# scalar-labs/jepsen

Measured on AMD Instinct MI355X. Metric: history ops verified/sec (node), independent cas-register 10k keys, 1/2/4/8 GPU, higher is better.
Workload: dtype int64

## Files before the change

include/jh.h:

```cpp
#ifndef JH_H
#define JH_H

#include <stddef.h>
#include <stdint.h>

#ifdef __cplusplus
extern "C" {
#endif

#define JH_ABI_VERSION 8

#define JH_OK            0
#define JH_EINVAL        1
#define JH_EUNSUPPORTED  2
#define JH_EDEVICE       3
#define JH_ENOMEM        4

#define JH_TYPE_INVOKE 0
#define JH_TYPE_OK     1
#define JH_TYPE_FAIL   2
#define JH_TYPE_INFO   3

#define JH_F_READ  0
#define JH_F_WRITE 1
// ... 48 lines not shown
#define JH_LIN_INTERN_PER_KEY  4
#define JH_LIN_NO_HELPERS      8
#define JH_LIN_HELPERS_NOW    16
#define JH_LIN_PHASE1_ONLY    32
#define JH_LIN_SKIP_PHASE1    64
#define JH_LIN_NO_HANDOVER   128
#define JH_LIN_STREAM        256
#define JH_LIN_NO_RESUME     512
#define JH_LIN_EXACT_COUNT  1024
#define JH_EXPLORED_UNCOUNTED (-3)
#define JH_LIN_NO_SPEC      2048
#define JH_LIN_SPEC_FIRST   4096
#define JH_LIN_HELP_STALL   8192
#define JH_LIN_NO_TAKEOVER  16384
#define JH_LIN_TAKEOVER     32768

typedef struct jh_lin_opts {
    int64_t init_value;
    int64_t budget;
    int64_t stream;
    int32_t algorithm;
    int32_t flags;
    int64_t quick_budget;
    int64_t phase2_budget;
    int32_t helpers;
    int32_t helper_late_us;
    int32_t xw_waves;
    int32_t p2_waves_per_cu;
    int32_t lean_waves;
    int32_t wide_waves;
// ... 328 lines not shown
```

jepsen_amd/_abi.py:

```python
import ctypes as C

JH_ABI_VERSION = 8

JH_OK, JH_EINVAL, JH_EUNSUPPORTED, JH_EDEVICE, JH_ENOMEM = 0, 1, 2, 3, 4
TYPE_INVOKE, TYPE_OK, TYPE_FAIL, TYPE_INFO = 0, 1, 2, 3
F_READ, F_WRITE, F_CAS, F_ADD = 0, 1, 2, 3
F_ENQUEUE, F_DEQUEUE, F_DRAIN = 4, 5, 6
F_FIRST_INTERNED = 16
NIL = -(1 << 63)

VALID, UNKNOWN, INVALID = 0, 1, 2

CAUSES = {
    0: None,
    1: "budget",
    2: "window",
    3: "double-invoke",
    4: "orphan-completion",
    5: "unsupported-f",
    6: "nil-value",
    7: "overflow",
    8: "states",
    9: "deferred",
    10: "multiple-writes",
# ... 25 lines not shown

ALGO_COMPETITION, ALGO_WGL, ALGO_LINEAR = 0, 1, 2
ALGORITHMS = {"competition": ALGO_COMPETITION, "wgl": ALGO_WGL, "linear": ALGO_LINEAR}
LIN_BFS_ONLY, LIN_GEN_JUMP, LIN_INTERN_PER_KEY, LIN_NO_HELPERS, LIN_HELPERS_NOW = 1, 2, 4, 8, 16
LIN_PHASE1_ONLY, LIN_SKIP_PHASE1 = 32, 64
LIN_NO_HANDOVER = 128
LIN_STREAM = 256
LIN_NO_RESUME = 512
LIN_EXACT_COUNT = 1024
EXPLORED_UNCOUNTED = -3
LIN_NO_SPEC = 2048
LIN_SPEC_FIRST = 4096
LIN_HELP_STALL = 8192
LIN_NO_TAKEOVER = 16384
LIN_TAKEOVER = 32768
CAUSE_DEFERRED = 9


class JhLinOpts(C.Structure):
    _fields_ = [("init_value", C.c_int64), ("budget", C.c_int64), ("stream", C.c_int64),
                ("algorithm", C.c_int32), ("flags", C.c_int32),
                ("quick_budget", C.c_int64), ("phase2_budget", C.c_int64),
                ("helpers", C.c_int32), ("helper_late_us", C.c_int32),
                ("xw_waves", C.c_int32), ("p2_waves_per_cu", C.c_int32),
                ("lean_waves", C.c_int32), ("wide_waves", C.c_int32),
                ("handover_min", C.c_int32), ("p1_waves_per_cu", C.c_int32),
                ("bfs_wgs", C.c_int32), ("helper_stall_min", C.c_int32)]


VERDICT_FIELDS = ("valid", "cause", "fail_entry", "explored", "previous_ok", "last_op", "analyzer")
# ... 223 lines not shown
```

jepsen_amd/csrc/jh_lin.hip:

```cpp
#include "jh_internal.h"
#include <hipcub/hipcub.hpp>
#include <algorithm>
#include <type_traits>
#include "lin/lin_common.h"

namespace {

constexpr int F_READ = 0, F_WRITE = 1, F_CAS = 2, F_OTHER = 4;
constexpr int T_INVOKE = 0, T_OK = 1, T_FAIL = 2, T_INFO = 3;
constexpr uint64_t VIOL_NONE = ~0ULL;
#ifndef JH_LDS_TBL
#define JH_LDS_TBL 0
#endif
constexpr int LDS_TBL = JH_LDS_TBL;
#ifdef JH_STEP_PROF
#define PROF_MARK(v) const unsigned long long v = __builtin_amdgcn_s_memtime()
#define PROF_ADD(acc, a, b) acc += (b) - (a)
#else
#define PROF_MARK(v)
#define PROF_ADD(acc, a, b)
#endif
#ifdef JH_DFS_STATS
#define DFS_STAT(x) x
#else
// ... 59 lines not shown
struct RangeOut {
    long long vmin, vmax;
    long long pmax;
    int unkeyed_client;
    int bad_value;
    int smax;
    int pad;
};

__device__ __forceinline__ int f_code(int64_t f) {
    return f == JH_F_READ ? F_READ : f == JH_F_WRITE ? F_WRITE : f == JH_F_CAS ? F_CAS : F_OTHER;
}

__global__ void __launch_bounds__(256) k_range(const int64_t *__restrict__ proc, const int64_t *__restrict__ f,
                        const int64_t *__restrict__ key, const int64_t *__restrict__ v1,
                        const int64_t *__restrict__ v2, int64_t n, int keyed, RangeOut *out) {
    long long lo = LLONG_MAX, hi = LLONG_MIN, pm = -1;
    int unk = 0;
    for (int64_t r = blockIdx.x * (int64_t)blockDim.x + threadIdx.x; r < n;
         r += (int64_t)gridDim.x * blockDim.x) {
        int64_t p = proc[r];
        if (p < 0) continue;
        pm = max(pm, (long long)p);
        if (keyed && key && key[r] < 0) unk = 1;
        const int fc = f_code(f[r]);
        if (fc <= F_CAS) {
            int64_t a = v1[r];
            if (a != JH_NIL) { lo = min(lo, (long long)a); hi = max(hi, (long long)a); }
            if (fc == F_CAS) {
                int64_t b = v2[r];
                if (b != JH_NIL) { lo = min(lo, (long long)b); hi = max(hi, (long long)b); }
            }
        }
    }
    __shared__ long long sh[4];
    __shared__ int shi[4];
    lo = block_reduce256(lo, RedMin(), sh);
    hi = block_reduce256(hi, RedMax(), sh);
    pm = block_reduce256(pm, RedMax(), sh);
// ... 24 lines not shown
    while (a < b) {
        int64_t m = (a + b) >> 1;
        if (sk[m] < (uint32_t)k) a = m + 1; else b = m;
    }
    off[k] = (uint32_t)a;
    if (k < K) {
        int64_t a2 = a, b2 = n;
        while (a2 < b2) {
            int64_t m = (a2 + b2) >> 1;
            if (sk[m] <= (uint32_t)k) a2 = m + 1; else b2 = m;
        }
        atomicMax(&ro->smax, (int)(a2 - a));
    }
}

__global__ void k_gather(const int64_t *__restrict__ proc, const int64_t *__restrict__ type,
                         const int64_t *__restrict__ f, const int64_t *__restrict__ v1,
                         const int64_t *__restrict__ v2, const uint32_t *__restrict__ rows,
                         int64_t m, long long vmin, Rec *__restrict__ rec) {
    for (int64_t p = blockIdx.x * (int64_t)blockDim.x + threadIdx.x; p < m;
         p += (int64_t)gridDim.x * blockDim.x) {
        uint32_t r = rows[p];
        Rec x;
        int64_t pr = proc[r];
        x.proc = pr < 0 ? -1 : (int32_t)pr;
        x.type = (uint8_t)type[r];
        x.f = (uint8_t)f_code(f[r]);
        x.pad = 0;
        int64_t a = v1[r], b = v2[r];
        x.v1 = a == JH_NIL ? 0 : (int32_t)(a - vmin + 1);
        x.v2 = b == JH_NIL ? 0 : (int32_t)(b - vmin + 1);
        if (x.f > F_CAS) { x.v1 = 0; x.v2 = 0; }
        rec[p] = x;
    }
}

__global__ void __launch_bounds__(256) k_pair(const Rec *__restrict__ rec, const uint32_t *__restrict__ sk,
                                              const uint32_t *__restrict__ off, int64_t m,
                                              int32_t *__restrict__ pair,
                                              unsigned long long *__restrict__ viol) {
    const int lane = threadIdx.x & 63;
    const int64_t nw = (int64_t)gridDim.x * 4;
    for (int64_t wv = (int64_t)blockIdx.x * 4 + (threadIdx.x >> 6); wv * 64 < m; wv += nw) {
        const int64_t base = wv * 64, p = base + lane;
        int32_t xp = -1, xt = T_INFO;
        uint32_t k = 0;
        if (p < m) { const Rec x = rec[p]; xp = x.proc; xt = x.type; k = sk[p]; }
        const bool inv = p < m && xp >= 0 && xt == T_INVOKE;
        const int64_t end = inv ? (int64_t)off[k + 1] : 0;
        bool open = inv && end > p + 1;
        int64_t got = -1;
        int gtype = 0;
        for (int64_t wb = base; wb < m; wb += 64) {
            if (!__ballot(open)) break;
            const int64_t j = wb + lane;
            int32_t yp = -1, yt = T_INFO;
            uint32_t yk = 0xFFFFFFFFu;
            if (j < m) { const Rec y = rec[j]; yp = y.proc; yt = y.type; yk = sk[j]; }
            uint64_t todo = __ballot(open);
            while (todo) {
                const int l = __builtin_ctzll(todo);
                const int32_t pl = __builtin_amdgcn_readlane(xp, l);
                const uint32_t kl = (uint32_t)__builtin_amdgcn_readlane((int)k, l);
// ... 10 lines not shown
                        got = wb + b; gtype = (int)((cinv >> b) & 1); open = false;
                    }
                }
            }
            if (open && wb + 64 >= end) open = false;
        }
        if (got >= 0) {
            if (gtype) atomicMin(&viol[k], ((unsigned long long)got << 4) | JH_CAUSE_DOUBLE_INVOKE);
            else { pair[p] = (int32_t)got; pair[got] = (int32_t)p; }
        }
    }
}

__global__ void k_orphan(const Rec *__restrict__ rec, const uint32_t *__restrict__ sk,
                         int64_t m, const int32_t *__restrict__ pair,
                         unsigned long long *__restrict__ viol) {
    for (int64_t p = blockIdx.x * (int64_t)blockDim.x + threadIdx.x; p < m;
         p += (int64_t)gridDim.x * blockDim.x) {
        Rec x = rec[p];
        if (x.proc < 0 || (x.type != T_OK && x.type != T_FAIL)) continue;
        if (pair[p] < 0) atomicMin(&viol[sk[p]], ((unsigned long long)p << 4) | JH_CAUSE_ORPHAN);
    }
}

struct DfsArgs {
    const Rec *rec;
    const int32_t *pair;
    const uint32_t *off;
    const uint32_t *rows;
    const unsigned long long *viol;
    int32_t *rank;
    const int32_t *list;
    int32_t n_list;
    int32_t *queue;
    jh_key_verdict *out;
// ... 1757 lines not shown
struct TblArgs {
    KeySrc src;
    int64_t K;
    KeyMeta *meta;
    char *arena;
    unsigned long long *bump;
    jh_key_verdict *out;
    int32_t *list;
    int32_t *n_list;
    int32_t *list_w;
    int32_t *n_list_w;
    int32_t *list_x;
    int32_t *n_list_x;
    unsigned long long *xw_max;
    int32_t states8;
};

__global__ void __launch_bounds__(256) k_key_tables(TblArgs A) {
    const int lane = threadIdx.x & 63;
    const int64_t nw = (int64_t)gridDim.x * 4;
    for (int64_t key = (int64_t)blockIdx.x * 4 + (threadIdx.x >> 6); key < A.K; key += nw) {
        KeyInfo K;
        jh_key_verdict v;
        bool need = key_pass1(A.src, (int)key, lane, K, v);
        const bool long_key = K.n_ok >= COMPACT_MAX_OK || K.n_ops > 65535;
        if (need) {
            int maxw = 65;
            if (!long_key && K.sumW <= 64LL * K.n_ok) {
                unsigned long long off = 0;
                if (lane == 0) off = atomicAdd(A.bump, (unsigned long long)tblc_bytes(K));
                off = (unsigned long long)rfl64(__shfl(off, 0));
                maxw = key_fill_c<false>(A.src, K, lane, A.arena + off);
                if (maxw <= 64 && lane == 0) {
                    KeyMeta m;
                    m.off = off; m.n_ops = K.n_ops; m.n_ok = K.n_ok; m.maxw = maxw;
                    m.pad = (int32_t)min(K.sumW, (long long)0x7FFFFFFE);
                    A.meta[key] = m;
                    if (A.states8 && maxw <= 40) A.list[atomicAdd(A.n_list, 1)] = (int32_t)key;
                    else A.list_w[atomicAdd(A.n_list_w, 1)] = (int32_t)key;
                }
            }
            if (maxw > 64 && lane == 0) {
                KeyMeta m;
                m.off = 0; m.n_ops = K.n_ops; m.n_ok = K.n_ok; m.maxw = -1; m.pad = (int32_t)K.sumW;
                A.meta[key] = m;
                A.list_x[atomicAdd(A.n_list_x, 1)] = (int32_t)key;
                atomicMax(A.xw_max, (unsigned long long)xw_bytes(K.n_ops, K.n_ok, K.sumW));
            }
        }
        if (!need && lane == 0) A.out[key] = v;
    }
}

template <class M, bool LEAN, bool WL = false, bool STREAM = false, bool HO = false>
__device__ __forceinline__ void lin_dfs_waves(const DfsArgs &A) {
    const int lane = threadIdx.x;
    const size_t wv = (size_t)(blockIdx.x - A.wave_off);
    uint64_t *memo = A.memo + wv * A.memo_cap * 2;
    Frame *stack = A.stack + wv * A.stack_cap;
    uint64_t *stage = (uint64_t *)(A.scratch + wv * A.scratch_bytes);
    unsigned long long my_probes = 0;
    const int n_list = A.n_list_dev ? *A.n_list_dev : A.n_list;
    if (n_list < A.n_min || (A.n_max > 0 && n_list > A.n_max)) return;
    const unsigned long long t_begin = __builtin_amdgcn_s_memtime();
    bool spanned = false;
// ... 3605 lines not shown
    EV_EARLY_END = 11,
    EV_HELP_END = 12, EV_P3_START = 13,
};

struct KeyPartition {
    uint32_t *kA, *kB, *rA, *rB;
    uint32_t *off;
};
KeyPartition partition_buffers(jh_ctx *ctx, int64_t n) {
    KeyPartition p{};
    p.kA = ctx->ws<uint32_t>(WS_KEYS_A, n); p.kB = ctx->ws<uint32_t>(WS_KEYS_B, n);
    p.rA = ctx->ws<uint32_t>(WS_ROWS_A, n); p.rB = ctx->ws<uint32_t>(WS_ROWS_B, n);
    return p;
}
void partition_by_key(jh_ctx *ctx, KeyPartition &p, const int64_t *key, int64_t n, int64_t K, bool keyed,
                      RangeOut *ro, hipStream_t st) {
    if (n > 0)
        k_keys<<<grid_for(n, 256), 256, 0, st>>>(keyed ? key : nullptr, n, K, keyed ? 1 : 0, p.kA, p.rA);
    const int endbit = bits_for((uint64_t)K);
    size_t tb = 0;
    HIP_TRY(hipcub::DeviceRadixSort::SortPairs(nullptr, tb, p.kA, p.kB, p.rA, p.rB, (int)n, 0, endbit, st));
    void *tmp = ctx->ws<char>(WS_SORT_TMP, tb);
    HIP_TRY(hipcub::DeviceRadixSort::SortPairs(tmp, tb, p.kA, p.kB, p.rA, p.rB, (int)n, 0, endbit, st));
    if (!p.off) p.off = ctx->ws<uint32_t>(WS_SEG_OFF, K + 2);
    k_seg_off<<<grid_for(K + 1, 256), 256, 0, st>>>(p.kB, n, K, p.off, ro);
}

struct BfsSizes {
    uint32_t set_cap, q_cap;
};
BfsSizes bfs_table_sizes(int64_t reach_cap) {
    uint32_t set_cap = 1u << 12;
    while ((int64_t)set_cap < 2 * reach_cap && set_cap < (1u << 30)) set_cap <<= 1;
    const uint32_t q_cap = (uint32_t)std::min<int64_t>(reach_cap + 64, (int64_t)1 << 30);
    return BfsSizes{set_cap, q_cap};
}

struct LinRun {
    jh_ctx *ctx = nullptr;
    const jh_history *dh = nullptr;
// ... 2 lines not shown
    jh_key_verdict *out_dev = nullptr;
    jh_summary *sum = nullptr;
    hipStream_t st = nullptr;
    const LinCfgReq *cfgreq = nullptr;
    int64_t n = 0, K = 0, budget = 0, init = 0;
    int32_t lflags = 0;
    bool linear_mode = false;

    RangeOut *ro = nullptr;
    long long vmin = 0, vmax = 0, n_states = 0;
    bool per_key_values = false;
    int init_state = 0;
    uint32_t *kB = nullptr, *rB = nullptr, *off = nullptr;
    int64_t m = 0;
    int smax = 1;
    Rec *rec = nullptr;
    int32_t *pair = nullptr;
    unsigned long long *viol = nullptr;
    int32_t *rank = nullptr;

    uint32_t gen_span = 0;
    bool clear_memo = false;

    const uint32_t memo_cap1 = 1u << 16;
    int64_t quick = 0;
    int waves1 = 0;
    uint32_t stack_cap = 0;
    uint64_t scr_bytes = 0, scr_bytes_h = 0, scr_bytes_bfs = 0;
    uint64_t *memo = nullptr;
    Frame *stack = nullptr;
// ... 29 lines not shown
    int n_unres = 0;
    bool use_wg = false, wg_race = false, stream_p2 = false;
    int wg2 = 0, n_help = 0;
    BfsArgs c{};
    DfsArgs b{};
    WgArgs wr{}, wh{};
    unsigned long long *seq_start = nullptr;
    uint32_t *seq_stall = nullptr;
    int p2_per_cu = P2_LEAN_PER_CU;
    bool p2_m = true, bfs_only = false;

    KeySrc key_src() const { return KeySrc{rec, pair, off, rB, viol, rank, q + Q_FLAGS}; }

    void prepare();
    void prep_ranges();
    void prep_records();
    void intern_per_key();
    void memo_generation();
    void phase1_tables();
    void phase1_args();
    void phase1_resume();
    void phase2_budgets();
    void ensure_lds_attrs();
    void prep_xw(const int32_t *qw);
    void prep_wide();
    void launch_wide(hipStream_t sw, bool p2);
    WgArgs build_wg(int wg_cus, int32_t *wg_claim, int32_t *wg_queue, bool all_cus = false);
    void prep_race(int nd_all, int nd_l);
    void race_bfs(int nd_all);
    int race_helper_count(int nd_l);
    uint64_t *race_lean_sizing(int nd_l, int help_cus);
    void race_helpers(int nd_l);
    void race_lean_args(int nd_l, uint64_t *memo2);
    void timeline_tables(bool wide);
    DfsArgs phase1_wide_args() const;
    DfsArgs phase3_lean_args() const;
    DfsArgs phase3_wide_args() const;
    void launch_phase3_lean(int waves, hipStream_t s);
    void entry_lists(bool live);
    void record_no_heavy_keys();
    void run_streaming();
    void run_phase1();
    void sort_deferred();
// ... 11 lines not shown
    void diag_defer_timeline();
    void diag_acc_trace();
    void diag_ws_report();
    void diag_xw_prof();
    void diag_summary();
};

}

#include "lin/lin_diag.h"

namespace {

void LinRun::prep_ranges() {
    ro = ctx->ws<RangeOut>(WS_MISC, 1);
    RangeOut ro_init{LLONG_MAX, LLONG_MIN, -1, 0, 0, 0, 0};
    HIP_TRY(hipMemcpyAsync(ro, &ro_init, sizeof ro_init, hipMemcpyHostToDevice, st));
    if (n > 0)
        k_range<<<grid_for(n, 256, 4096), 256, 0, st>>>(dh->process, dh->f, keyed ? dh->key : nullptr,
                                                        dh->value, dh->value2, n, keyed ? 1 : 0, ro);
    RangeOut rh;
    HIP_TRY(hipMemcpyAsync(&rh, ro, sizeof rh, hipMemcpyDeviceToHost, st));
    HIP_TRY(hipStreamSynchronize(st));
    if (keyed && rh.unkeyed_client)
        throw_jh(JH_EUNSUPPORTED, "client ops whose :value is not an independent tuple");
    if (rh.pmax > INT32_MAX) throw_jh(JH_EUNSUPPORTED, "process ids beyond int32");
    vmin = rh.vmin; vmax = rh.vmax;
    if (init != JH_NIL) { vmin = std::min<long long>(vmin, init); vmax = std::max<long long>(vmax, init); }
    if (vmin > vmax) { vmin = 0; vmax = 0; }
    per_key_values = (unsigned long long)(vmax - vmin) >= (unsigned long long)(RQ_EMPTY - 3) ||
                     (lflags & JH_LIN_INTERN_PER_KEY) != 0;
    init_state = init == JH_NIL ? 0 : per_key_values ? 1 : (int)(init - vmin + 1);
    n_states = vmax - vmin + 2;
}

void LinRun::prep_records() {
    rec = ctx->ws<Rec>(WS_REC, m);
    pair = ctx->ws<int32_t>(WS_PAIR, m);
    viol = ctx->ws<unsigned long long>(WS_VIOL, K);
    rank = ctx->ws<int32_t>(WS_RANK, m);
    HIP_TRY(hipMemsetAsync(viol, 0xFF, sizeof(unsigned long long) * K, st));
    if (m > 0) {
        HIP_TRY(hipMemsetAsync(pair, 0xFF, sizeof(int32_t) * m, st));
        k_gather<<<grid_for(m, 256), 256, 0, st>>>(dh->process, dh->type, dh->f, dh->value, dh->value2,
                                                   rB, m, vmin, rec);
        k_pair<<<grid_for((m + 63) / 64, 4, 16384), 256, 0, st>>>(rec, kB, off, m, pair, viol);
        k_orphan<<<grid_for(m, 256), 256, 0, st>>>(rec, kB, m, pair, viol);
    }
}

void LinRun::intern_per_key() {
    const int64_t n2 = 2 * m;
    if (n2 >= (1LL << 32) - 1) throw_jh(JH_EUNSUPPORTED, "too many entries for per-key value interning");
    const int endbit = bits_for((uint64_t)K);
    uint64_t *iu = ctx->ws<uint64_t>(WS_IV_U, 2 * n2);
    uint32_t *ix = ctx->ws<uint32_t>(WS_IV_IDX, 3 * n2);
    uint32_t *ik = ctx->ws<uint32_t>(WS_IV_KEY, 2 * n2);
    uint32_t *rinit = ctx->ws<uint32_t>(WS_IV_RINIT, K + 1);
    unsigned int *maxid = (unsigned int *)ctx->ws<uint32_t>(WS_IV_MAX, 4);
    uint32_t *flag = ik + n2;
    k_ival<<<grid_for(n2, 256), 256, 0, st>>>(dh->value, dh->value2, dh->f, rB, m, iu, ix);
    size_t tb1 = 0, tb2 = 0, tb3 = 0;
// ... 10 lines not shown
    HIP_TRY(hipcub::DeviceScan::InclusiveSum(itmp, tb3, flag, flag, (int)n2, st));
    const uint64_t init_u = (uint64_t)init ^ (1ULL << 63);
    HIP_TRY(hipMemsetAsync(rinit, 0, sizeof(uint32_t) * (K + 1), st));
    HIP_TRY(hipMemsetAsync(maxid, 0, sizeof(unsigned int), st));
    if (init != JH_NIL) k_iinit<<<grid_for(n2, 256), 256, 0, st>>>(idx2, iu, kB, off, flag, n2, init_u, rinit);
    k_iassign<<<grid_for(n2, 256), 256, 0, st>>>(idx2, iu, kB, off, flag, n2, init != JH_NIL ? 1 : 0, init_u,
                                                 rinit, rec, viol, maxid);
    unsigned int mh = 0;
    HIP_TRY(hipMemcpyAsync(&mh, maxid, sizeof mh, hipMemcpyDeviceToHost, st));
    HIP_TRY(hipStreamSynchronize(st));
    n_states = (long long)std::max<unsigned int>(mh, init != JH_NIL ? 1u : 0u) + 1;
}

void LinRun::prepare() {
    prep_ranges();
    KeyPartition kp = partition_buffers(ctx, n);
    partition_by_key(ctx, kp, dh->key, n, K, keyed, ro, st);
    kB = kp.kB; rB = kp.rB; off = kp.off;
    uint32_t m_keyed = 0;
    RangeOut rh;
    HIP_TRY(hipMemcpyAsync(&m_keyed, off + K, sizeof m_keyed, hipMemcpyDeviceToHost, st));
    HIP_TRY(hipMemcpyAsync(&rh, ro, sizeof rh, hipMemcpyDeviceToHost, st));
    HIP_TRY(hipStreamSynchronize(st));
    m = m_keyed;
    smax = std::max(rh.smax, 1);
    prep_records();
    if (per_key_values && m > 0) intern_per_key();
}

void LinRun::memo_generation() {
    gen_span = (uint32_t)(3 * K + 3);
    clear_memo = false;
    if (lflags & JH_LIN_GEN_JUMP) ctx->gen_base = (1u << GEN_BITS) - 2;
    if ((uint64_t)ctx->gen_base + gen_span >= (1u << GEN_BITS) - 1) {
        ctx->gen_base = 0;
#ifndef JH_NO_WRAP_CLEAR
        clear_memo = true;
#endif
    }
}
// ... 6 lines not shown
    if (opts && opts->p1_waves_per_cu > 0) p1_per_cu = std::min(p1_per_cu, (int)opts->p1_waves_per_cu);
    waves1 = (int)std::min<int64_t>(K, (int64_t)ctx->n_cu * p1_per_cu);
    memo = ctx->ws<uint64_t>(WS_MEMO, (size_t)waves1 * memo_cap1 * 2, true);
    if (clear_memo) HIP_TRY(hipMemsetAsync(memo, 0, ctx->bufs[WS_MEMO].bytes, st));
    stack_cap = (uint32_t)smax + 2;
    stack = ctx->ws<Frame>(WS_STACK, (size_t)waves1 * stack_cap);
    scr_bytes = MemoQ::SLOTS * 8;
    scr_bytes_h = MemoH::SLOTS * 8;
    scr_bytes_bfs = (((uint64_t)smax * 84 + 4096) + 255) & ~255ULL;
    scr = ctx->ws<char>(WS_SCRATCH, (size_t)waves1 * scr_bytes);
    q = ctx->ws<int32_t>(WS_QUEUE, Q_WORDS);
    list = ctx->ws<int32_t>(WS_STATS, K);
    defer = ctx->ws<int32_t>(WS_DEFER, 3 * (size_t)(K + 1));
    defer_l = defer + (K + 1); defer_w = defer + 2 * (K + 1);
    d64 = ctx->ws<uint64_t>(WS_DEFER64, 3 * (size_t)(K + 1));
    HIP_TRY(hipMemsetAsync(q, 0, Q_WORDS * sizeof(int32_t), st));
    HIP_TRY(hipMemsetAsync(q + Q_T_WIDE, 0xFF, 2 * sizeof(int32_t), st));
    for (int w : {Q_T_BFS, Q_T_LEAN, Q_T_XW, Q_T_P1}) HIP_TRY(hipMemsetAsync(q + w, 0xFF, 2 * sizeof(int32_t), st));

    meta = ctx->ws<KeyMeta>(WS_META, K);
    arena = ctx->ws<char>(WS_ARENA, (size_t)m * 8 + (size_t)K * 32 + 256);
    TblArgs ta{};
    ta.src = key_src();
    ta.K = K; ta.meta = meta; ta.arena = arena; ta.bump = (unsigned long long *)(q + Q_BUMP);
    list_w = ctx->ws<int32_t>(WS_LIST_W, K);
    ta.out = out_dev; ta.list = list; ta.n_list = q + Q_N_LIST; ta.list_w = list_w; ta.n_list_w = q + Q_N_LIST_W;
    list_x = ctx->ws<int32_t>(WS_LIST_X, K);
    ta.list_x = list_x; ta.n_list_x = q + Q_N_LIST_X; ta.xw_max = (unsigned long long *)(q + Q_XW_MAX);
    ta.states8 = n_states <= 256 ? 1 : 0;
    k_key_tables<<<(unsigned)std::min<int64_t>((K + 3) / 4, 8192), 256, 0, st>>>(ta);

    list1 = list;
    if (!tune_env("JH_NO_LPT") && K > 1) {
        uint32_t *cost = ctx->ws<uint32_t>(WS_LCOST, 2 * K);
        int32_t *lv = ctx->ws<int32_t>(WS_LSORT, 2 * K);
        k_list_cost<<<grid_for(K, 256, 4096), 256, 0, st>>>(list, q + Q_N_LIST, meta, K, cost, lv);
        size_t tbl = 0;
        HIP_TRY(hipcub::DeviceRadixSort::SortPairsDescending(nullptr, tbl, cost, cost + K, lv, lv + K, (int)K, 0, 32, st));
        HIP_TRY(hipcub::DeviceRadixSort::SortPairsDescending(ctx->ws<char>(WS_LTMP, tbl), tbl, cost, cost + K, lv,
                                                             lv + K, (int)K, 0, 32, st));
        list1 = lv + K;
    }
}

void LinRun::phase1_args() {
// ... 222 lines not shown
    }
    wa.pend = ctx->ws<uint64_t>(WS_WG_PEND, (size_t)n_wg * 2 * work_cap);
    if (!ctx->lds_attr_wg) {
        HIP_TRY(hipFuncSetAttribute((const void *)k_lin_wg, hipFuncAttributeMaxDynamicSharedMemorySize, WG_LDS));
        ctx->lds_attr_wg = true;
    }
    return wa;
}

void LinRun::prep_race(int nd_all, int nd_l) {
    race_bfs(nd_all);
    const int help_cus = race_helper_count(nd_l);
    uint64_t *memo2 = race_lean_sizing(nd_l, help_cus);
    race_helpers(nd_l);
    race_lean_args(nd_l, memo2);
}

void LinRun::race_bfs(int nd_all) {
    claim = ctx->ws<int32_t>(WS_CLAIM, K);
    HIP_TRY(hipMemsetAsync(claim, 0, (size_t)K * sizeof(int32_t), st));
    HIP_TRY(hipMemsetAsync(q + Q_QUEUE, 0, sizeof(int32_t), st));
    HIP_TRY(hipMemsetAsync(q + Q_UNRES, 0, sizeof(int32_t), st));
    HIP_TRY(hipMemsetAsync(q + Q_P2_QUEUE, 0, sizeof(int32_t), st));

    uint32_t ncap = 1u << 22;
    if (const char *e = tune_env("JH_BFS_NODES")) ncap = (uint32_t)std::max(1 << 16, std::min(1 << 26, atoi(e)));
    const int64_t reach_cap = std::max<int64_t>(budget + 1, ncap);
    const BfsSizes sz = bfs_table_sizes(reach_cap);
    const uint32_t set_cap = sz.set_cap, q_cap = sz.q_cap;
    uint32_t hcap = 1u << 16;
    while (hcap < 2 * (uint64_t)ncap) hcap <<= 1;
    const uint32_t lcap = (uint32_t)smax + 2;
    const int bfs_cus = std::max(1, nd_all > 2000 && nd_all <= 4000 ? ctx->n_cu / 4
                                                                      : std::min(96, ctx->n_cu * 3 / 8));
    wg2 = std::min(nd_all, tune_env("JH_BFS_CUS") ? std::max(1, atoi(tune_env("JH_BFS_CUS"))) :
                           opts && opts->bfs_wgs > 0 ? std::min(opts->bfs_wgs, ctx->n_cu - 16) : bfs_cus);
    const uint64_t per_bfs = (uint64_t)set_cap * 8 + 4ULL * q_cap * 8 + scr_bytes_bfs + (uint64_t)ncap * 8 +
                             (uint64_t)lcap * 4 + (uint64_t)hcap * 16 + (uint64_t)ncap * 4 + ((uint64_t)ncap / 32 + 1) * 4 +
// ... 73 lines not shown
    }
    return memo2;
}

void LinRun::race_helpers(int nd_l) {
    wr = WgArgs{};
    if (wg_race && nd_l > 0) wr = build_wg(std::max(1, ctx->n_cu - wg2), claim, q + Q_P2_QUEUE);
    wh = WgArgs{};
    seq_start = nullptr;
    seq_stall = nullptr;
    if (n_help <= 0) return;
    const bool spec_on = !(lflags & JH_LIN_NO_SPEC) && !(tune_env("JH_SPEC") && !atoi(tune_env("JH_SPEC")));
    wh = build_wg(n_help, claim, nullptr, spec_on);
    seq_start = ctx->ws<unsigned long long>(WS_HELP_START, K);
    int32_t *taken = ctx->ws<int32_t>(WS_HELP_TAKEN, 2 * (size_t)K);
    HIP_TRY(hipMemsetAsync(seq_start, 0, (size_t)K * sizeof(unsigned long long), st));
    HIP_TRY(hipMemsetAsync(taken, 0, 2 * (size_t)K * sizeof(int32_t), st));
    seq_stall = (uint32_t *)(taken + K);
    wh.seq_start = seq_start; wh.seq_exit = q + Q_SEQ_EXIT; wh.seq_waves = waves2; wh.taken = taken;
    wh.mains_live = q + Q_MAINS;
    uint64_t late_us = HELPER_LATE_US;
    if (opts && opts->helper_late_us > 0) late_us = (uint64_t)opts->helper_late_us;
    if (lflags & JH_LIN_HELPERS_NOW) late_us = 0;
    wh.late_ticks = late_us * 100;
    const bool by_time = JH_HELP_BY_ORDER || (opts && opts->helper_late_us > 0) ||
                         (lflags & (JH_LIN_HELPERS_NOW | JH_LIN_HELP_STALL));
    wh.stall = by_time ? nullptr : seq_stall;
    wh.stall_min = opts && opts->helper_stall_min > 0 ? (uint32_t)opts->helper_stall_min : HELPER_STALL_MIN;
    if (spec_on) {
        wh.spec = ctx->ws<SpecSlot>(WS_SPEC, SPEC_SLOTS);
        HIP_TRY(hipMemsetAsync(wh.spec, 0, sizeof(SpecSlot) * SPEC_SLOTS, st));
        wh.spec_res_cap = SPEC_RES_CAP;
        wh.spec_res = ctx->ws<uint64_t>(WS_SPEC_RES, (size_t)n_wg * SPEC_RES_CAP);
        wh.spec_min = 512; wh.spec_mult = 32; wh.spec_dist = 128;
        wh.spec_q = q + Q_SPEC;
        wh.spec_first = (lflags & JH_LIN_SPEC_FIRST) ? 1 : 0;
        wh.n_mains = std::min(n_wg, HELPER_MAINS);
        if (const char *e = tune_env("JH_SPEC_SERVERS")) wh.n_mains = std::max(1, n_wg - std::max(0, atoi(e)));
        if (const char *e = tune_env("JH_SPEC_MIN")) wh.spec_min = (uint32_t)std::max(1, atoi(e));
        if (const char *e = tune_env("JH_SPEC_MULT")) wh.spec_mult = (uint32_t)std::max(1, atoi(e));
        if (const char *e = tune_env("JH_SPEC_DIST")) wh.spec_dist = (uint32_t)std::max(1, atoi(e));
    }
}

void LinRun::race_lean_args(int nd_l, uint64_t *memo2) {
    const int wmax = std::max(waves2, waves3);
// ... 7 lines not shown
    b.defer_list = defer3; b.defer_count = q + Q_DEFER3;
    b.defer64 = nullptr; b.defer_kind = nullptr; b.defer_kind_count = nullptr;
    b.memo = memo2; b.memo_cap = cap2l; b.stack = stack2; b.scratch = scr2; b.scratch_bytes = scr_bytes_h;
    b.budget = split3 ? p2 : budget;
    b.budget_full = split3 && cap2l == cap2 ? budget : 0;
    b.gen_base = ctx->gen_base + (uint32_t)K + 1;
    b.dbg = dbg ? dbg + 16 * 256 : nullptr; b.claim = claim;
    b.probes = (unsigned long long *)(q + Q_PROBES_SEQ);
    b.seq_start = seq_start; b.exit_count = seq_start ? q + Q_SEQ_EXIT : nullptr;
    b.stamp_progress = seq_start && (lflags & JH_LIN_HELP_STALL) ? 1 : 0;
    b.stall = seq_stall;
    b.defer_time = nullptr;
    b.handoff = nullptr;
    if (n_help > 0 && a.rs_off && waves2 > 0 && (lflags & JH_LIN_TAKEOVER) && !(lflags & JH_LIN_NO_TAKEOVER)) {
        int32_t *ho = ctx->ws<int32_t>(WS_HANDOFF, K);
        HIP_TRY(hipMemsetAsync(ho, 0, (size_t)K * sizeof(int32_t), st));
        b.handoff = ho;
        b.hlog_cap = 32768;
        b.hlog = ctx->ws<uint32_t>(WS_RS_LOG2, (size_t)wmax * b.hlog_cap);
        wh.d.handoff = ho;
    }
}

void LinRun::timeline_tables(bool wide) {
    if (!defer_times) return;
    unsigned long long *tl = ctx->ws<unsigned long long>(WS_TL, TL_W * (size_t)K);
    HIP_TRY(hipMemsetAsync(tl, 0, TL_W * sizeof(unsigned long long) * K, st));
    c.tl = tl; b.tl = tl;
    if (wide) bw.tl = tl;
    if (n_help > 0) wh.d.tl = tl;
}
// ... 552 lines not shown
```

Measured before the change: 261.3 million.

## Fuse per-key record gather, pairing and table build into one wave kernel

Adds k_key_build, a one-wave-per-key kernel that builds the records, pairs invocations with completions, checks violations and emits the key tables from LDS, for keys up to a segment cap. The separate gather/pair/orphan/tables kernels now run only on longer keys, or not at all. k_range also writes the key and row arrays for the partition step, and the many small hipMemsetAsync calls are batched into one fill kernel plus a queue-init kernel. The aim is to cut launch overhead and global-memory round trips during preparation, at the cost of a large and complex new code path that has to reproduce the old pairing semantics exactly.

Result: faster. 265.9 million (median of 6 runs) (+1.7%).

```diff
diff --git a/include/jh.h b/include/jh.h
--- a/include/jh.h
+++ b/include/jh.h
@@ -86,6 +86,8 @@
 #define JH_LIN_HELP_STALL   8192
 #define JH_LIN_NO_TAKEOVER  16384
 #define JH_LIN_TAKEOVER     32768
+#define JH_LIN_PREP_SPLIT   65536
+#define JH_LIN_PREP_CAP     1024
 
 typedef struct jh_lin_opts {
     int64_t init_value;
diff --git a/jepsen_amd/_abi.py b/jepsen_amd/_abi.py
--- a/jepsen_amd/_abi.py
+++ b/jepsen_amd/_abi.py
@@ -63,6 +63,8 @@
 LIN_HELP_STALL = 8192
 LIN_NO_TAKEOVER = 16384
 LIN_TAKEOVER = 32768
+LIN_PREP_SPLIT = 65536
+LIN_PREP_CAP = 1024
 CAUSE_DEFERRED = 9
 
 
diff --git a/jepsen_amd/csrc/jh_lin.hip b/jepsen_amd/csrc/jh_lin.hip
--- a/jepsen_amd/csrc/jh_lin.hip
+++ b/jepsen_amd/csrc/jh_lin.hip
@@ -97,15 +97,19 @@
 
 __global__ void __launch_bounds__(256) k_range(const int64_t *__restrict__ proc, const int64_t *__restrict__ f,
                         const int64_t *__restrict__ key, const int64_t *__restrict__ v1,
-                        const int64_t *__restrict__ v2, int64_t n, int keyed, RangeOut *out) {
+                        const int64_t *__restrict__ v2, int64_t n, int keyed, RangeOut *out,
+                        int64_t K, uint32_t *__restrict__ k32, uint32_t *__restrict__ r32) {
     long long lo = LLONG_MAX, hi = LLONG_MIN, pm = -1;
     int unk = 0;
     for (int64_t r = blockIdx.x * (int64_t)blockDim.x + threadIdx.x; r < n;
          r += (int64_t)gridDim.x * blockDim.x) {
         int64_t p = proc[r];
+        const int64_t kr = keyed ? (key ? key[r] : -1) : 0;
+        k32[r] = (kr >= 0 && kr < K) ? (uint32_t)kr : (uint32_t)K;
+        r32[r] = (uint32_t)r;
         if (p < 0) continue;
         pm = max(pm, (long long)p);
-        if (keyed && key && key[r] < 0) unk = 1;
+        if (keyed && key && kr < 0) unk = 1;
         const int fc = f_code(f[r]);
         if (fc <= F_CAS) {
             int64_t a = v1[r];
@@ -160,12 +164,18 @@
     }
 }
 
+__device__ __forceinline__ bool seg_longer(const uint32_t *off, uint32_t k, int64_t min_len) {
+    return (int64_t)(off[k + 1] - off[k]) > min_len;
+}
+
 __global__ void k_gather(const int64_t *__restrict__ proc, const int64_t *__restrict__ type,
                          const int64_t *__restrict__ f, const int64_t *__restrict__ v1,
                          const int64_t *__restrict__ v2, const uint32_t *__restrict__ rows,
-                         int64_t m, long long vmin, Rec *__restrict__ rec) {
+                         int64_t m, long long vmin, Rec *__restrict__ rec,
+                         const uint32_t *__restrict__ sk, const uint32_t *__restrict__ off, int64_t min_len) {
     for (int64_t p = blockIdx.x * (int64_t)blockDim.x + threadIdx.x; p < m;
          p += (int64_t)gridDim.x * blockDim.x) {
+        if (min_len >= 0 && !seg_longer(off, sk[p], min_len)) continue;
         uint32_t r = rows[p];
         Rec x;
         int64_t pr = proc[r];
@@ -184,7 +194,7 @@
 __global__ void __launch_bounds__(256) k_pair(const Rec *__restrict__ rec, const uint32_t *__restrict__ sk,
                                               const uint32_t *__restrict__ off, int64_t m,
                                               int32_t *__restrict__ pair,
-                                              unsigned long long *__restrict__ viol) {
+                                              unsigned long long *__restrict__ viol, int64_t min_len) {
     const int lane = threadIdx.x & 63;
     const int64_t nw = (int64_t)gridDim.x * 4;
     for (int64_t wv = (int64_t)blockIdx.x * 4 + (threadIdx.x >> 6); wv * 64 < m; wv += nw) {
@@ -192,7 +202,7 @@
         int32_t xp = -1, xt = T_INFO;
         uint32_t k = 0;
         if (p < m) { const Rec x = rec[p]; xp = x.proc; xt = x.type; k = sk[p]; }
-        const bool inv = p < m && xp >= 0 && xt == T_INVOKE;
+        const bool inv = p < m && xp >= 0 && xt == T_INVOKE && (min_len < 0 || seg_longer(off, k, min_len));
         const int64_t end = inv ? (int64_t)off[k + 1] : 0;
         bool open = inv && end > p + 1;
         int64_t got = -1;
@@ -233,11 +243,12 @@
 
 __global__ void k_orphan(const Rec *__restrict__ rec, const uint32_t *__restrict__ sk,
                          int64_t m, const int32_t *__restrict__ pair,
-                         unsigned long long *__restrict__ viol) {
+                         unsigned long long *__restrict__ viol, const uint32_t *__restrict__ off, int64_t min_len) {
     for (int64_t p = blockIdx.x * (int64_t)blockDim.x + threadIdx.x; p < m;
          p += (int64_t)gridDim.x * blockDim.x) {
         Rec x = rec[p];
         if (x.proc < 0 || (x.type != T_OK && x.type != T_FAIL)) continue;
+        if (min_len >= 0 && !seg_longer(off, sk[p], min_len)) continue;
         if (pair[p] < 0) atomicMin(&viol[sk[p]], ((unsigned long long)p << 4) | JH_CAUSE_ORPHAN);
     }
 }
@@ -2025,12 +2036,14 @@
     int32_t *n_list_x;
     unsigned long long *xw_max;
     int32_t states8;
+    int64_t min_len;
 };
 
 __global__ void __launch_bounds__(256) k_key_tables(TblArgs A) {
     const int lane = threadIdx.x & 63;
     const int64_t nw = (int64_t)gridDim.x * 4;
     for (int64_t key = (int64_t)blockIdx.x * 4 + (threadIdx.x >> 6); key < A.K; key += nw) {
+        if (A.min_len >= 0 && !seg_longer(A.src.off, (uint32_t)key, A.min_len)) continue;
         KeyInfo K;
         jh_key_verdict v;
         bool need = key_pass1(A.src, (int)key, lane, K, v);
@@ -2060,6 +2073,295 @@
             }
         }
         if (!need && lane == 0) A.out[key] = v;
+    }
+}
+
+constexpr int KB_CAP = JH_LIN_PREP_CAP;
+constexpr int KB_GATHER = 4;
+static_assert(KB_CAP < COMPACT_MAX_OK && KB_CAP < 32768 && KB_CAP < (int)T_MASK, "segment-local ranks and pairs");
+
+struct BuildArgs {
+    TblArgs t;
+    const int64_t *proc, *type, *f, *v1, *v2;
+    long long vmin;
+    Rec *rec;
+    int32_t *pair;
+    unsigned long long *viol;
+};
+
+struct KbLds {
+    int32_t pr[KB_CAP];
+    uint16_t v1[KB_CAP], v2[KB_CAP];
+    int16_t pw[KB_CAP];
+    int16_t ri[KB_CAP];
+    uint8_t tf[KB_CAP];
+};
+
+__device__ int kb_scan_back(const KbLds &sh, int pl, int base, int lane) {
+    for (int b = base - 64; b >= 0; b -= 64) {
+        const int ty = sh.tf[b + lane] & 31;
+        const uint64_t m = ballot(sh.pr[b + lane] == pl && ty != T_INFO);
+        if (m) {
+            const int h = 63 - __builtin_clzll(m);
+            return readlane(ty, h) == T_INVOKE ? b + h : -1;
+        }
+    }
+    return -1;
+}
+
+__device__ __forceinline__ void kb_settle(jh_key_verdict *out, int64_t key, int valid, int cause, long long explored) {
+    jh_key_verdict v{};
+    v.valid = valid; v.cause = cause; v.fail_entry = -1; v.explored = explored;
+    out[key] = v;
+}
+
+__device__ __forceinline__ uint32_t kb_rq(int f, int v1c, int v2c) {
+    return f == F_READ ? ((uint32_t)v1c | ((uint32_t)v1c << 16))
+         : f == F_WRITE ? (RQ_ANY | ((uint32_t)v1c << 16))
+         : ((uint32_t)v1c | ((uint32_t)v2c << 16));
+}
+
+__device__ __forceinline__ int wave_sum(int x) {
+    for (int o = 32; o > 0; o >>= 1) x += __shfl_xor(x, o);
+    return x;
+}
+
+__global__ void __launch_bounds__(64) k_key_build(BuildArgs B) {
+    __shared__ KbLds sh;
+    const int lane = threadIdx.x;
+    const uint64_t lt = (1ULL << lane) - 1;
+    const TblArgs &A = B.t;
+    const KeySrc &S = A.src;
+    const int64_t k8 = (A.K + 7) / 8;
+    for (int64_t b = blockIdx.x; b < 8 * k8; b += gridDim.x) {
+        const int64_t key = (b & 7) * k8 + (b >> 3);
+        if (key >= A.K) continue;
+        const uint32_t s0 = S.off[key], s1 = S.off[key + 1];
+        if (s1 - s0 > (uint32_t)KB_CAP) continue;
+        const int len = (int)(s1 - s0);
+        if (len == 0) {
+            if (lane == 0) { B.viol[key] = VIOL_NONE; kb_settle(A.out, key, JH_VALID, 0, -1); }
+            continue;
+        }
+        wave_sync();
+        for (int base = 0; base < len; base += 64 * KB_GATHER) {
+            uint32_t r[KB_GATHER];
+            int64_t cp[KB_GATHER], ct[KB_GATHER], cf[KB_GATHER], ca[KB_GATHER], cb[KB_GATHER];
+#pragma unroll
+            for (int g = 0; g < KB_GATHER; g++) r[g] = S.rows[s0 + min(base + g * 64 + lane, len - 1)];
+#pragma unroll
+            for (int g = 0; g < KB_GATHER; g++) {
+                cp[g] = B.proc[r[g]]; ct[g] = B.type[r[g]]; cf[g] = B.f[r[g]]; ca[g] = B.v1[r[g]]; cb[g] = B.v2[r[g]];
+            }
+#pragma unroll
+            for (int g = 0; g < KB_GATHER; g++) {
+                const int i = base + g * 64 + lane;
+                if (i >= len) continue;
+                Rec x;
+                x.proc = cp[g] < 0 ? -1 : (int32_t)cp[g];
+                x.type = (uint8_t)ct[g];
+                x.f = (uint8_t)f_code(cf[g]);
+                x.pad = 0;
+                x.v1 = ca[g] == JH_NIL ? 0 : (int32_t)(ca[g] - B.vmin + 1);
+                x.v2 = cb[g] == JH_NIL ? 0 : (int32_t)(cb[g] - B.vmin + 1);
+                if (x.f > F_CAS) { x.v1 = 0; x.v2 = 0; }
+                B.rec[s0 + i] = x;
+                sh.pr[i] = x.proc;
+                sh.v1[i] = (uint16_t)x.v1; sh.v2[i] = (uint16_t)x.v2;
+                sh.tf[i] = (uint8_t)((x.type > 31 ? 31 : x.type) | (x.f << 5));
+                sh.pw[i] = -1;
+            }
+        }
+        wave_sync();
+        unsigned long long vi = VIOL_NONE;
+        {
+            int tproc = 0, tpos = -1;
+            bool recycled = false;
+            int victim = 0;
+            for (int base = 0; base < len; base += 64) {
+                const int i = base + lane;
+                const bool valid = i < len;
+                const int xp = valid ? sh.pr[i] : -1;
+                const int xt = valid ? sh.tf[i] & 31 : T_INFO;
+                const bool cand = xp >= 0 && xt != T_INFO;
+                const uint64_t invm = ballot(cand && xt == T_INVOKE);
+                uint64_t mygrp = 0;
+                int mypred0 = -1;
+                uint64_t todo = ballot(cand);
+                while (todo) {
+                    const int pl = readlane(xp, __builtin_ctzll(todo));
+                    const bool mine = cand && xp == pl;
+                    const uint64_t grp = ballot(mine);
+                    todo &= ~grp;
+                    const uint64_t hit = ballot(tpos >= 0 && tproc == pl);
+                    int pred0 = -1;
+                    if (hit) {
+                        const int hl = __builtin_ctzll(hit);
+                        pred0 = readlane(tpos, hl);
+                        if (lane == hl) tpos = -1;
+                    } else if (recycled) {
+                        pred0 = kb_scan_back(sh, pl, base, lane);
+                    }
+                    if (mine) { mygrp = grp; mypred0 = pred0; }
+                    const int last = 63 - __builtin_clzll(grp);
+                    if ((invm >> last) & 1) {
+                        const uint64_t fr = ~ballot(tpos >= 0);
+                        int slot;
+                        if (fr) slot = __builtin_ctzll(fr);
+                        else { slot = victim; victim = (victim + 1) & 63; recycled = true; }
+                        if (lane == slot) { tproc = pl; tpos = base + last; }
+                    }
+                }
+                if (cand) {
+                    const uint64_t below = mygrp & lt;
+                    int pred = mypred0;
+                    bool pinv = mypred0 >= 0;
+                    if (below) {
+                        const int bl = 63 - __builtin_clzll(below);
+                        pred = base + bl; pinv = ((invm >> bl) & 1) != 0;
+                    }
+                    if (pinv && xt == T_INVOKE)
+                        vi = min(vi, ((unsigned long long)(s0 + i) << 4) | JH_CAUSE_DOUBLE_INVOKE);
+                    else if (pinv) { sh.pw[i] = (int16_t)pred; sh.pw[pred] = (int16_t)i; }
+                    else if (xt == T_OK || xt == T_FAIL)
+                        vi = min(vi, ((unsigned long long)(s0 + i) << 4) | JH_CAUSE_ORPHAN);
+                }
+            }
+            for (int o = 32; o > 0; o >>= 1) vi = min(vi, (unsigned long long)__shfl_xor((long long)vi, o));
+        }
+        wave_sync();
+        for (int base = 0; base < len; base += 64) {
+            const int i = base + lane;
+            if (i < len) {
+                const int q = sh.pw[i];
+                B.pair[s0 + i] = q < 0 ? -1 : (int32_t)(s0 + q);
+            }
+        }
+        if (lane == 0) B.viol[key] = vi;
+        if (vi != VIOL_NONE) {
+            if (lane == 0) kb_settle(A.out, key, JH_UNKNOWN, (int)(vi & 15), 0);
+            continue;
+        }
+        int n_ops = 0, n_ok = 0, n_crash = 0, badf = 0;
+        int acc_ok = 0, acc_crash = 0, acc_w = 0;
+        for (int base = 0; base < len; base += 64) {
+            const int i = base + lane;
+            const bool valid = i < len;
+            int xp = -1, xt = 0, xf = 0, xv1 = 0, xv2 = 0, q = -1;
+            if (valid) {
+                const int tf = sh.tf[i];
+                xp = sh.pr[i]; xt = tf & 31; xf = tf >> 5; xv1 = sh.v1[i]; xv2 = sh.v2[i]; q = sh.pw[i];
+            }
+            int yt = 0, yf = 0, yv1 = 0, yv2 = 0;
+            if (q >= 0) {
+                const int tf = sh.tf[q];
+                yt = tf & 31; yf = tf >> 5; yv1 = sh.v1[q]; yv2 = sh.v2[q];
+            }
+            const bool inv = xp >= 0 && xt == T_INVOKE;
+            const bool c_ok = inv && q >= 0 && yt == T_OK;
+            const bool c_fail = inv && q >= 0 && yt == T_FAIL;
+            int v1c = xv1;
+            if (c_ok && xv1 == 0 && (xf != F_CAS || xv2 == 0)) v1c = yv1;
+            const bool kept = inv && !c_fail && !(xf == F_READ && (!c_ok || v1c == 0));
+            bool ret = false;
+            if (xp >= 0 && xt == T_OK && q >= 0) {
+                int iv1 = yv1;
+                if (iv1 == 0 && (yf != F_CAS || yv2 == 0)) iv1 = xv1;
+                ret = !(yf == F_READ && iv1 == 0);
+            }
+            const uint64_t bi = ballot(kept), br = ballot(ret);
+            const int my_op = n_ops + mbcnt(bi);
+            const int a = n_ok + mbcnt(br);
+            const int rk = kept ? my_op : (ret ? -(a + 2) : -1);
+            if (valid) { S.rank[s0 + i] = rk; sh.pr[i] = rk; sh.ri[i] = (int16_t)(ret ? q : -1); }
+            badf |= (int)(ballot(kept && xf > F_CAS) != 0);
+            const bool crash = kept && !c_ok;
+            n_crash += __popcll(ballot(crash));
+            acc_ok += (kept && c_ok) ? a : 0;
+            acc_crash += crash ? a : 0;
+            if (ret) acc_w = max(acc_w, my_op - a);
+            n_ops += __popcll(bi);
+            n_ok += __popcll(br);
+        }
+        const int sum_a_ok = wave_sum(acc_ok), sum_a_crash = wave_sum(acc_crash);
+        int maxw = acc_w;
+        for (int o = 32; o > 0; o >>= 1) maxw = max(maxw, __shfl_xor(maxw, o));
+        KeyInfo K;
+        K.s0 = s0; K.s1 = s1; K.n_ops = n_ops; K.n_ok = n_ok;
+        K.sumW = (long long)n_ok * (n_ok + 1) / 2 - sum_a_ok + (long long)n_crash * n_ok - sum_a_crash;
+        const int cause = badf ? JH_CAUSE_BAD_F : n_ok == 0 ? 0 : K.sumW > (long long)JH_MAX_WINDOW * n_ok ? JH_CAUSE_WINDOW : -1;
+        if (cause >= 0) {
+            if (lane == 0) kb_settle(A.out, key, cause ? JH_UNKNOWN : JH_VALID, cause, 0);
+            continue;
+        }
+        if (maxw > 64) {
+            if (lane == 0) {
+                KeyMeta m;
+                m.off = 0; m.n_ops = n_ops; m.n_ok = n_ok; m.maxw = -1; m.pad = (int32_t)K.sumW;
+                A.meta[key] = m;
+                A.list_x[atomicAdd(A.n_list_x, 1)] = (int32_t)key;
+                atomicMax(A.xw_max, (unsigned long long)xw_bytes(n_ops, n_ok, K.sumW));
+            }
+            continue;
+        }
+        unsigned long long off = 0;
+        if (lane == 0) off = atomicAdd(A.bump, (unsigned long long)tblc_bytes(K));
+        off = (unsigned long long)rfl64(__shfl(off, 0));
+        OpC *ops = (OpC *)(A.arena + off);
+        Lay *lay = (Lay *)(A.arena + off + tblc_ops_bytes(K));
+        wave_sync();
+        int nok = 0, since = 0;
+        for (int base = 0; base < len; base += 64) {
+            const int i = base + lane;
+            const int rk = i < len ? sh.pr[i] : -1;
+            const bool kept = rk >= 0, ret = rk <= -2;
+            const uint64_t bi = ballot(kept), br = ballot(ret);
+            if (kept) {
+                const int xf = sh.tf[i] >> 5, q = sh.pw[i];
+                int rr = -1, v1c = sh.v1[i], v2c = sh.v2[i];
+                if (q >= 0 && (sh.tf[q] & 31) == T_OK) {
+                    rr = -(sh.pr[q] + 2);
+                    if (xf == F_CAS) { if (v1c == 0 && v2c == 0) { v1c = sh.v1[q]; v2c = sh.v2[q]; } }
+                    else if (v1c == 0) v1c = sh.v1[q];
+                }
+                const int a = nok + mbcnt(br);
+                OpC o;
+                o.rq = kb_rq(xf, v1c, v2c);
+                o.fa = (uint32_t)xf | ((uint32_t)a << 2) | ((uint32_t)(rr + 1) << 16);
+                ops[rk] = o;
+            }
+            if (ret) {
+                const int t = -(rk + 2), q = sh.pw[i];
+                const uint64_t rb = br & lt;
+                int c;
+                if (rb) c = __popcll(bi & lt & ~((2ULL << (63 - __builtin_clzll(rb))) - 1));
+                else c = since + __popcll(bi & lt);
+                int nested = 0;
+                for (int p2 = q + 1; p2 < i; p2 += 4) {
+                    const int r0 = sh.ri[p2], r1 = sh.ri[min(p2 + 1, i)], r2 = sh.ri[min(p2 + 2, i)], r3 = sh.ri[min(p2 + 3, i)];
+                    nested += (r0 > q) + (p2 + 1 < i && r1 > q) + (p2 + 2 < i && r2 > q) + (p2 + 3 < i && r3 > q);
+                }
+                const int r = sh.pr[q] - t + nested;
+                const int yf = sh.tf[q] >> 5;
+                int v1c = sh.v1[q], v2c = sh.v2[q];
+                if (yf == F_CAS) { if (v1c == 0 && v2c == 0) { v1c = sh.v1[i]; v2c = sh.v2[i]; } }
+                else if (v1c == 0) v1c = sh.v1[i];
+                Lay e;
+                e.rq = kb_rq(yf, v1c, v2c);
+                e.hi = (uint32_t)r | ((uint32_t)c << 6);
+                lay[t] = e;
+            }
+            since = br ? __popcll(bi & ~((2ULL << (63 - __builtin_clzll(br))) - 1)) : since + __popcll(bi);
+            nok += __popcll(br);
+        }
+        if (lane == 0) {
+            KeyMeta m;
+            m.off = off; m.n_ops = n_ops; m.n_ok = n_ok; m.maxw = maxw;
+            m.pad = (int32_t)min(K.sumW, (long long)0x7FFFFFFE);
+            A.meta[key] = m;
+            if (A.states8 && maxw <= 40) A.list[atomicAdd(A.n_list, 1)] = (int32_t)key;
+            else A.list_w[atomicAdd(A.n_list_w, 1)] = (int32_t)key;
+        }
     }
 }
 
@@ -5695,8 +5997,8 @@
     return p;
 }
 void partition_by_key(jh_ctx *ctx, KeyPartition &p, const int64_t *key, int64_t n, int64_t K, bool keyed,
-                      RangeOut *ro, hipStream_t st) {
-    if (n > 0)
+                      RangeOut *ro, hipStream_t st, bool have_pairs = false) {
+    if (n > 0 && !have_pairs)
         k_keys<<<grid_for(n, 256), 256, 0, st>>>(keyed ? key : nullptr, n, K, keyed ? 1 : 0, p.kA, p.rA);
     const int endbit = bits_for((uint64_t)K);
     size_t tb = 0;
@@ -5705,6 +6007,30 @@
     HIP_TRY(hipcub::DeviceRadixSort::SortPairs(tmp, tb, p.kA, p.kB, p.rA, p.rB, (int)n, 0, endbit, st));
     if (!p.off) p.off = ctx->ws<uint32_t>(WS_SEG_OFF, K + 2);
     k_seg_off<<<grid_for(K + 1, 256), 256, 0, st>>>(p.kB, n, K, p.off, ro);
+}
+
+__global__ void k_init_q(int32_t *q) {
+    const int w = threadIdx.x;
+    if (w >= Q_WORDS) return;
+    bool start = false;
+    for (int s : {Q_T_WIDE, Q_T_BFS, Q_T_LEAN, Q_T_XW, Q_T_P1}) start |= w == s || w == s + 1;
+    q[w] = start ? -1 : 0;
+}
+
+struct FillJob {
+    uint32_t *p;
+    uint64_t words;
+    uint32_t val;
+    uint32_t pad;
+};
+struct FillBatch {
+    FillJob j[8];
+    int n;
+};
+__global__ void __launch_bounds__(256) k_fill(FillBatch F) {
+    for (int i = 0; i < F.n; i++)
+        for (uint64_t w = blockIdx.x * 256ull + threadIdx.x; w < F.j[i].words; w += gridDim.x * 256ull)
+            F.j[i].p[w] = F.j[i].val;
 }
 
 struct BfsSizes {
@@ -5737,6 +6063,11 @@
     uint32_t *kB = nullptr, *rB = nullptr, *off = nullptr;
     int64_t m = 0;
     int smax = 1;
+    KeyPartition kp{};
+    FillBatch fills{};
+    const RangeOut ro_init{LLONG_MAX, LLONG_MIN, -1, 0, 0, 0, 0};
+    bool fused = false;
+    int64_t split_min = -1;
     Rec *rec = nullptr;
     int32_t *pair = nullptr;
     unsigned long long *viol = nullptr;
@@ -5796,6 +6127,7 @@
 
     void prepare();
     void prep_ranges();
+    void use_ranges(const RangeOut &rh);
     void prep_records();
     void intern_per_key();
     void memo_generation();
@@ -5809,6 +6141,8 @@
     void launch_wide(hipStream_t sw, bool p2);
     WgArgs build_wg(int wg_cus, int32_t *wg_claim, int32_t *wg_queue, bool all_cus = false);
     void prep_race(int nd_all, int nd_l);
+    void fill_later(void *p, size_t bytes, uint32_t val);
+    void flush_fills();
     void race_bfs(int nd_all);
     int race_helper_count(int nd_l);
     uint64_t *race_lean_sizing(int nd_l, int help_cus);
@@ -5850,14 +6184,14 @@
 
 void LinRun::prep_ranges() {
     ro = ctx->ws<RangeOut>(WS_MISC, 1);
-    RangeOut ro_init{LLONG_MAX, LLONG_MIN, -1, 0, 0, 0, 0};
+    kp = partition_buffers(ctx, n);
     HIP_TRY(hipMemcpyAsync(ro, &ro_init, sizeof ro_init, hipMemcpyHostToDevice, st));
     if (n > 0)
         k_range<<<grid_for(n, 256, 4096), 256, 0, st>>>(dh->process, dh->f, keyed ? dh->key : nullptr,
-                                                        dh->value, dh->value2, n, keyed ? 1 : 0, ro);
-    RangeOut rh;
-    HIP_TRY(hipMemcpyAsync(&rh, ro, sizeof rh, hipMemcpyDeviceToHost, st));
-    HIP_TRY(hipStreamSynchronize(st));
+                                                        dh->value, dh->value2, n, keyed ? 1 : 0, ro, K, kp.kA, kp.rA);
+}
+
+void LinRun::use_ranges(const RangeOut &rh) {
     if (keyed && rh.unkeyed_client)
         throw_jh(JH_EUNSUPPORTED, "client ops whose :value is not an independent tuple");
     if (rh.pmax > INT32_MAX) throw_jh(JH_EUNSUPPORTED, "process ids beyond int32");
@@ -5868,6 +6202,8 @@
                      (lflags & JH_LIN_INTERN_PER_KEY) != 0;
     init_state = init == JH_NIL ? 0 : per_key_values ? 1 : (int)(init - vmin + 1);
     n_states = vmax - vmin + 2;
+    fused = !per_key_values && !(lflags & JH_LIN_PREP_SPLIT);
+    split_min = !fused ? -1 : smax > KB_CAP ? KB_CAP : INT64_MAX;
 }
 
 void LinRun::prep_records() {
@@ -5875,13 +6211,14 @@
     pair = ctx->ws<int32_t>(WS_PAIR, m);
     viol = ctx->ws<unsigned long long>(WS_VIOL, K);
     rank = ctx->ws<int32_t>(WS_RANK, m);
+    if (split_min == INT64_MAX) return;
     HIP_TRY(hipMemsetAsync(viol, 0xFF, sizeof(unsigned long long) * K, st));
     if (m > 0) {
         HIP_TRY(hipMemsetAsync(pair, 0xFF, sizeof(int32_t) * m, st));
         k_gather<<<grid_for(m, 256), 256, 0, st>>>(dh->process, dh->type, dh->f, dh->value, dh->value2,
-                                                   rB, m, vmin, rec);
-        k_pair<<<grid_for((m + 63) / 64, 4, 16384), 256, 0, st>>>(rec, kB, off, m, pair, viol);
-        k_orphan<<<grid_for(m, 256), 256, 0, st>>>(rec, kB, m, pair, viol);
+                                                   rB, m, vmin, rec, kB, off, split_min);
+        k_pair<<<grid_for((m + 63) / 64, 4, 16384), 256, 0, st>>>(rec, kB, off, m, pair, viol, split_min);
+        k_orphan<<<grid_for(m, 256), 256, 0, st>>>(rec, kB, m, pair, viol, off, split_min);
     }
 }
 
@@ -5922,8 +6259,7 @@
 
 void LinRun::prepare() {
     prep_ranges();
-    KeyPartition kp = partition_buffers(ctx, n);
-    partition_by_key(ctx, kp, dh->key, n, K, keyed, ro, st);
+    partition_by_key(ctx, kp, dh->key, n, K, keyed, ro, st, true);
     kB = kp.kB; rB = kp.rB; off = kp.off;
     uint32_t m_keyed = 0;
     RangeOut rh;
@@ -5932,6 +6268,7 @@
     HIP_TRY(hipStreamSynchronize(st));
     m = m_keyed;
     smax = std::max(rh.smax, 1);
+    use_ranges(rh);
     prep_records();
     if (per_key_values && m > 0) intern_per_key();
 }
@@ -5968,9 +6305,8 @@
     defer = ctx->ws<int32_t>(WS_DEFER, 3 * (size_t)(K + 1));
     defer_l = defer + (K + 1); defer_w = defer + 2 * (K + 1);
     d64 = ctx->ws<uint64_t>(WS_DEFER64, 3 * (size_t)(K + 1));
-    HIP_TRY(hipMemsetAsync(q, 0, Q_WORDS * sizeof(int32_t), st));
-    HIP_TRY(hipMemsetAsync(q + Q_T_WIDE, 0xFF, 2 * sizeof(int32_t), st));
-    for (int w : {Q_T_BFS, Q_T_LEAN, Q_T_XW, Q_T_P1}) HIP_TRY(hipMemsetAsync(q + w, 0xFF, 2 * sizeof(int32_t), st));
+    static_assert(Q_WORDS <= 128, "k_init_q: one thread per word");
+    k_init_q<<<1, 128, 0, st>>>(q);
 
     meta = ctx->ws<KeyMeta>(WS_META, K);
     arena = ctx->ws<char>(WS_ARENA, (size_t)m * 8 + (size_t)K * 32 + 256);
@@ -5982,7 +6318,16 @@
     list_x = ctx->ws<int32_t>(WS_LIST_X, K);
     ta.list_x = list_x; ta.n_list_x = q + Q_N_LIST_X; ta.xw_max = (unsigned long long *)(q + Q_XW_MAX);
     ta.states8 = n_states <= 256 ? 1 : 0;
-    k_key_tables<<<(unsigned)std::min<int64_t>((K + 3) / 4, 8192), 256, 0, st>>>(ta);
+    ta.min_len = split_min;
+    if (split_min != INT64_MAX)
+        k_key_tables<<<(unsigned)std::min<int64_t>((K + 3) / 4, 8192), 256, 0, st>>>(ta);
+    if (fused) {
+        BuildArgs ba{};
+        ba.t = ta;
+        ba.proc = dh->process; ba.type = dh->type; ba.f = dh->f; ba.v1 = dh->value; ba.v2 = dh->value2;
+        ba.vmin = vmin; ba.rec = rec; ba.pair = pair; ba.viol = viol;
+        k_key_build<<<(unsigned)std::min<int64_t>(K, 1 << 20), 64, 0, st>>>(ba);
+    }
 
     list1 = list;
     if (!tune_env("JH_NO_LPT") && K > 1) {
@@ -6235,14 +6580,28 @@
     uint64_t *memo2 = race_lean_sizing(nd_l, help_cus);
     race_helpers(nd_l);
     race_lean_args(nd_l, memo2);
+    flush_fills();
+}
+
+void LinRun::fill_later(void *p, size_t bytes, uint32_t val) {
+    if (bytes == 0) return;
+    if (fills.n == (int)(sizeof fills.j / sizeof fills.j[0])) flush_fills();
+    fills.j[fills.n++] = FillJob{(uint32_t *)p, bytes / 4, val, 0};
+}
+void LinRun::flush_fills() {
+    if (fills.n == 0) return;
+    uint64_t most = 0;
+    for (int i = 0; i < fills.n; i++) most = std::max(most, fills.j[i].words);
+    k_fill<<<(unsigned)std::min<uint64_t>((most + 255) / 256, 1024), 256, 0, st>>>(fills);
+    fills.n = 0;
 }
 
 void LinRun::race_bfs(int nd_all) {
     claim = ctx->ws<int32_t>(WS_CLAIM, K);
-    HIP_TRY(hipMemsetAsync(claim, 0, (size_t)K * sizeof(int32_t), st));
-    HIP_TRY(hipMemsetAsync(q + Q_QUEUE, 0, sizeof(int32_t), st));
-    HIP_TRY(hipMemsetAsync(q + Q_UNRES, 0, sizeof(int32_t), st));
-    HIP_TRY(hipMemsetAsync(q + Q_P2_QUEUE, 0, sizeof(int32_t), st));
+    fill_later(claim, (size_t)K * sizeof(int32_t), 0);
+    fill_later(q + Q_QUEUE, sizeof(int32_t), 0);
+    fill_later(q + Q_UNRES, sizeof(int32_t), 0);
+    fill_later(q + Q_P2_QUEUE, sizeof(int32_t), 0);
 
     uint32_t ncap = 1u << 22;
     if (const char *e = tune_env("JH_BFS_NODES")) ncap = (uint32_t)std::max(1 << 16, std::min(1 << 26, atoi(e)));
@@ -6346,8 +6705,8 @@
     wh = build_wg(n_help, claim, nullptr, spec_on);
     seq_start = ctx->ws<unsigned long long>(WS_HELP_START, K);
     int32_t *taken = ctx->ws<int32_t>(WS_HELP_TAKEN, 2 * (size_t)K);
-    HIP_TRY(hipMemsetAsync(seq_start, 0, (size_t)K * sizeof(unsigned long long), st));
-    HIP_TRY(hipMemsetAsync(taken, 0, 2 * (size_t)K * sizeof(int32_t), st));
+    fill_later(seq_start, (size_t)K * sizeof(unsigned long long), 0);
+    fill_later(taken, 2 * (size_t)K * sizeof(int32_t), 0);
     seq_stall = (uint32_t *)(taken + K);
     wh.seq_start = seq_start; wh.seq_exit = q + Q_SEQ_EXIT; wh.seq_waves = waves2; wh.taken = taken;
     wh.mains_live = q + Q_MAINS;
@@ -6361,7 +6720,8 @@
     wh.stall_min = opts && opts->helper_stall_min > 0 ? (uint32_t)opts->helper_stall_min : HELPER_STALL_MIN;
     if (spec_on) {
         wh.spec = ctx->ws<SpecSlot>(WS_SPEC, SPEC_SLOTS);
-        HIP_TRY(hipMemsetAsync(wh.spec, 0, sizeof(SpecSlot) * SPEC_SLOTS, st));
+        static_assert(sizeof(SpecSlot) % 4 == 0, "filled by words");
+        fill_later(wh.spec, sizeof(SpecSlot) * SPEC_SLOTS, 0);
         wh.spec_res_cap = SPEC_RES_CAP;
         wh.spec_res = ctx->ws<uint64_t>(WS_SPEC_RES, (size_t)n_wg * SPEC_RES_CAP);
         wh.spec_min = 512; wh.spec_mult = 32; wh.spec_dist = 128;
@@ -6399,7 +6759,7 @@
     b.handoff = nullptr;
     if (n_help > 0 && a.rs_off && waves2 > 0 && (lflags & JH_LIN_TAKEOVER) && !(lflags & JH_LIN_NO_TAKEOVER)) {
         int32_t *ho = ctx->ws<int32_t>(WS_HANDOFF, K);
-        HIP_TRY(hipMemsetAsync(ho, 0, (size_t)K * sizeof(int32_t), st));
+        fill_later(ho, (size_t)K * sizeof(int32_t), 0);
         b.handoff = ho;
         b.hlog_cap = 32768;
         b.hlog = ctx->ws<uint32_t>(WS_RS_LOG2, (size_t)wmax * b.hlog_cap);
```
